# chanchanchan97/ICAFusion

Measured on AMD Instinct MI355X. Metric: RGB/IR image-pairs/sec (two-stream forward + NMS), higher is better.
Workload: dtype bf16

## Files before the change

### icafusion_amd/csrc/api.hip

```cpp
#include "icaf_common.h"
#include <cstring>

namespace icaf {
std::string& last_error() {
    static thread_local std::string e;
    return e;
}
int fail(int code, const char* fmt, ...) {
    char buf[1024];
    va_list ap;
    va_start(ap, fmt);
    vsnprintf(buf, sizeof(buf), fmt, ap);
    va_end(ap);
    last_error() = buf;
    return code;
}
LibOptions g_opt;
}

using namespace icaf;

extern "C" const char* icaf_last_error(void) { return last_error().c_str(); }

extern "C" int icaf_set_option(const char* name, int value) {
    if (!name) return fail(ICAF_ERR_ARG, "icaf_set_option: null name");
    if (!strcmp(name, "detect_elementwise")) g_opt.detect_elementwise = value;
    else if (!strcmp(name, "attn_qsplit")) g_opt.attn_qsplit = value;
    else if (!strcmp(name, "sppf_vpb")) g_opt.sppf_vpb = value;
    else if (!strcmp(name, "letterbox_direct")) g_opt.letterbox_direct = value;
    else if (!strcmp(name, "index64")) g_opt.index64 = value;
    else if (!strcmp(name, "attn_stream")) g_opt.attn_stream = value;
    else if (!strcmp(name, "area_direct")) g_opt.area_direct = value;
    else return fail(ICAF_ERR_ARG, "icaf_set_option: unknown option '%s' (detect_elementwise, attn_qsplit, sppf_vpb, letterbox_direct, index64, attn_stream, area_direct)", name);
    return ICAF_OK;
}
extern "C" int icaf_version(void) { return 100; }

extern "C" int icaf_device_info(int* cu_count, int* lds_bytes, char* arch, int arch_len) {
    int dev = 0;
    ICAF_HIP(hipGetDevice(&dev));
    hipDeviceProp_t prop;
    ICAF_HIP(hipGetDeviceProperties(&prop, dev));
    if (cu_count) *cu_count = prop.multiProcessorCount;
    if (lds_bytes) *lds_bytes = (int)prop.sharedMemPerBlock;
    if (arch && arch_len > 0) {
        strncpy(arch, prop.gcnArchName, arch_len - 1);
        arch[arch_len - 1] = 0;
    }
    return ICAF_OK;
}

extern "C" int icaf_graph_begin(icaf_stream_t s) {
    ICAF_HIP(hipStreamBeginCapture(S(s), hipStreamCaptureModeThreadLocal));
    return ICAF_OK;
}
extern "C" int icaf_graph_end(icaf_stream_t s, void** graph_exec) {
    hipGraph_t graph = nullptr;
    ICAF_HIP(hipStreamEndCapture(S(s), &graph));
    hipGraphExec_t exec = nullptr;
    hipError_t e = hipGraphInstantiate(&exec, graph, nullptr, nullptr, 0);
    hipGraphDestroy(graph);
    if (e != hipSuccess) return fail(ICAF_ERR_HIP, "hipGraphInstantiate -> %s", hipGetErrorString(e));
    *graph_exec = (void*)exec;
    return ICAF_OK;
}
extern "C" int icaf_graph_launch(void* graph_exec, icaf_stream_t s) {
    ICAF_HIP(hipGraphLaunch((hipGraphExec_t)graph_exec, S(s)));
    return ICAF_OK;
}
extern "C" int icaf_graph_destroy(void* graph_exec) {
    if (graph_exec) ICAF_HIP(hipGraphExecDestroy((hipGraphExec_t)graph_exec));
    return ICAF_OK;
}
extern "C" int icaf_event_create(void** ev) {
    hipEvent_t e;
    ICAF_HIP(hipEventCreate(&e));
    *ev = (void*)e;
    return ICAF_OK;
}
extern "C" int icaf_event_record(void* ev, icaf_stream_t s) {
    ICAF_HIP(hipEventRecord((hipEvent_t)ev, S(s)));
    return ICAF_OK;
}
extern "C" int icaf_stream_wait_event(icaf_stream_t s, void* ev) {
    ICAF_HIP(hipStreamWaitEvent(S(s), (hipEvent_t)ev, 0));
    return ICAF_OK;
// ... 15 lines not shown
```

### icafusion_amd/csrc/dmff_wide.hip

```cpp
#include <type_traits>
#include "icaf_common.h"
#include "conv_common.h"

namespace icaf {

struct WideP {
    const void* x;
    const void* att;
    float* part;
    const float* x32;
    float* y32;
    void* qkv;
    void* y;
    const void* wqkv; const float* bqkv;
    const void* wo; const float* bo;
    const void* w1; const float* b1;
    const void* w2; const float* b2;
    const float* ln_a_g[2]; const float* ln_a_b[2];
    const float* ln_m_g; const float* ln_m_b;
    long long wqkv_gs, bqkv_gs, wo_gs, bo_gs, w1_gs, b1_gs, w2_gs, b2_gs, x_gs, y_gs;
    long long rows;
    int C, Kp, Kp4, hid, ldy;
    int qkv_npass;
    float eps_a, eps_m;
    float c_res_a[2], c_acc_a[2], c_res_m[2], c_acc_m[2];
};

constexpr int WROWS = 64;
constexpr int WDEPTH = 4;
template <int NW_, int SL_> struct WG {
    static constexpr int NW = NW_, SL = SL_;
    static constexpr int WT = 64 * NW;
    static constexpr int WPASS = 32 * NW;
    template <int DT> static constexpr int kstep() { return 32 / Elem<DT>::BYTES; }
    template <int DT> static constexpr int ksl() { return kstep<DT>() * SL; }
    template <int DT> static constexpr int nsl2() { return WPASS / ksl<DT>(); }
    static constexpr int TPR = WT / WROWS;
};
using WG8 = WG<8, 4>;
using WG4 = WG<4, 2>;

struct WCursor {
    const u32x4* base;
    int left, seg;
};

template <int WSL, class NEXT>
__device__ __forceinline__ void wfetch(u32x4 (&w)[WSL], WCursor& c, const NEXT& next) {
    if (c.left == 0) return;
#pragma unroll
    for (int k = 0; k < WSL; ++k) w[k] = c.base[k * 64];
    c.base += WSL * 64;
    if (--c.left == 0) { ++c.seg; next(c); }
}

template <int DT, int WSL, class NEXT>
__device__ __forceinline__ void wpass(f32x16 (&acc)[2], const unsigned char* A, int SA, int n, u32x4 (&wq)[WDEPTH][WSL], WCursor& c, const NEXT& next) {
    const int lane = threadIdx.x & 63, l31 = lane & 31, hi = lane >> 5;
    const unsigned char* a0 = A + (size_t)l31 * SA + hi * 16;
    const unsigned char* a1 = a0 + (size_t)32 * SA;
    for (int s = 0; s < n; s += WDEPTH) {
#pragma unroll
        for (int u = 0; u < WDEPTH; ++u) {
#pragma unroll
            for (int k = 0; k < WSL; ++k) {
                const int off = ((s + u) * WSL + k) * 32;
                const u32x4 x0 = *(const u32x4*)(a0 + off);
                const u32x4 x1 = *(const u32x4*)(a1 + off);
                mma_step<DT>(acc[0], wq[u][k], x0);
                mma_step<DT>(acc[1], wq[u][k], x1);
            }
            wfetch<WSL>(wq[u], c, next);
            __builtin_amdgcn_sched_barrier(0);
        }
    }
}

template <int DT, int TPR>
__device__ __forceinline__ void wide_tile_layernorm(unsigned char* tile, int S, int C, const float* __restrict__ gam, const float* __restrict__ bet, float eps) {
    using E = Elem<DT>;
    const int tid = threadIdx.x, row = tid / TPR, part = tid % TPR;
    const int nv = C / E::VEC;
    unsigned char* r = tile + (size_t)row * S;
    float s = 0.0f;
    for (int v = part; v < nv; v += TPR) {
        float t[E::VEC];
        unpack16<DT>(*(const u32x4*)(r + v * 16), t);
#pragma unroll
        for (int j = 0; j < E::VEC; ++j) s += t[j];
    }
    s += __shfl_xor(s, 1); s += __shfl_xor(s, 2);
    if constexpr (TPR == 8) s += __shfl_xor(s, 4);
    const float mean = s / (float)C;
    float q = 0.0f;
    for (int v = part; v < nv; v += TPR) {
        float t[E::VEC];
        unpack16<DT>(*(const u32x4*)(r + v * 16), t);
#pragma unroll
        for (int j = 0; j < E::VEC; ++j) { const float d = t[j] - mean; q += d * d; }
    }
    q += __shfl_xor(q, 1); q += __shfl_xor(q, 2);
    if constexpr (TPR == 8) q += __shfl_xor(q, 4);
    const float rstd = 1.0f / sqrtf(q / (float)C + eps);
    for (int v = part; v < nv; v += TPR) {
        float t[E::VEC], o[E::VEC];
        unpack16<DT>(*(const u32x4*)(r + v * 16), t);
#pragma unroll
        for (int j = 0; j < E::VEC; ++j) o[j] = (t[j] - mean) * rstd * gam[v * E::VEC + j] + bet[v * E::VEC + j];
        *(u32x4*)(r + v * 16) = pack16<DT>(o);
    }
}

__device__ __forceinline__ void wide_place(int bid, int& g, int& idx) { g = (bid & 7) >> 2; idx = (bid >> 3) * 4 + (bid & 3); }
template <int KS> __device__ __forceinline__ void wide_place_ks(int bid, int& g, int& ks, int& idx) {
    const int x = bid & 7, per = 4 / KS;
    g = x >> 2;
    ks = (x & 3) / per;
    idx = (bid >> 3) * per + (x & 3) % per;
}

template <int DT, class G = WG8>
__global__ __launch_bounds__(G::WT) void dmff_wide_ln_qkv_kernel(const WideP p) {
    using E = Elem<DT>;
    using T = typename E::type;
    constexpr int VEC = E::VEC, EB = E::BYTES;
    extern __shared__ __attribute__((aligned(16))) unsigned char smem[];
    const int C = p.C, SA = C * EB + 16;
    unsigned char* tile = smem;
    const int tid = threadIdx.x, lane = tid & 63, l31 = lane & 31, hi = lane >> 5;
    const int wn = __builtin_amdgcn_readfirstlane(tid >> 6);
    const int npass = p.qkv_npass;
    const int ngrp = 3 * (C / G::WPASS) / npass;
    const int ntiles = (int)((p.rows + WROWS - 1) / WROWS);
    int g, idx;
    wide_place(blockIdx.x, g, idx);
    if (idx >= ntiles * ngrp) return;
    const int tile_i = idx / ngrp, grp = idx - tile_i * ngrp;
    const long long r0 = (long long)tile_i * WROWS;
    const int ks_row = p.Kp / G::template kstep<DT>(), nsl = C / G::template ksl<DT>();

    const u32x4* wf = (const u32x4*)((const T*)p.wqkv + g * p.wqkv_gs) + lane;
    auto next = [&](WCursor& c) {
        if (c.seg >= npass) { c.left = 0; return; }
        c.base = wf + (long long)((grp * npass + c.seg) * G::NW + wn) * ks_row * 64;
        c.left = nsl;
    };
    WCursor cur; cur.seg = 0; next(cur);
    u32x4 wq[WDEPTH][G::SL];
#pragma unroll
    for (int u = 0; u < WDEPTH; ++u) wfetch<G::SL>(wq[u], cur, next);

    {
        const T* xg = (const T*)p.x + g * p.x_gs;
        const int nv = C / VEC;
        for (int i = tid; i < WROWS * nv; i += G::WT) {
            const int row = i / nv, v = i - row * nv;
            long long r = r0 + row;
            r = r < p.rows ? r : p.rows - 1;
            *(u32x4*)(tile + (size_t)row * SA + v * 16) = *(const u32x4*)(xg + r * C + v * VEC);
        }
    }
    lds_barrier();
    wide_tile_layernorm<DT, G::TPR>(tile, SA, C, p.ln_a_g[g], p.ln_a_b[g], p.eps_a);
    lds_barrier();

    const float* bias = p.bqkv + g * p.bqkv_gs;
    const int nout = 3 * C;
    T* out = (T*)p.qkv + (long long)g * p.rows * nout;
    for (int j = 0; j < npass; ++j) {
        f32x16 acc[2];
#pragma unroll
        for (int t = 0; t < 2; ++t)
#pragma unroll
            for (int r = 0; r < 16; ++r) acc[t][r] = 0.0f;
        wpass<DT, G::SL>(acc, tile, SA, nsl, wq, cur, next);
        const int nb = (grp * npass + j) * G::WPASS + wn * 32;
#pragma unroll
        for (int t = 0; t < 2; ++t) {
            const long long row = r0 + t * 32 + l31;
            if (row < p.rows) {
#pragma unroll
                for (int q = 0; q < 4; ++q) {
                    const int n = nb + 8 * q + 4 * hi;
                    const f32x4 b = *(const f32x4*)(bias + n);
                    *(typename Quad<DT>::type*)(out + row * nout + n) =
                        pack4<DT>(acc[t][4 * q] + b[0], acc[t][4 * q + 1] + b[1], acc[t][4 * q + 2] + b[2], acc[t][4 * q + 3] + b[3]);
                }
            }
        }
    }
}

template <int DT, int NPW, int KS = 1, class G = WG8, bool R32 = false>
__global__ __launch_bounds__(G::WT) void dmff_wide_proj_mlp_kernel(const WideP p) {
    using E = Elem<DT>;
    using T = typename E::type;
    constexpr int VEC = E::VEC, EB = E::BYTES;
    extern __shared__ __attribute__((aligned(16))) unsigned char smem[];
    const int C = p.C, SA = C * EB + 16;
    constexpr int WPASS = G::WPASS, WT = G::WT, NSL2 = G::template nsl2<DT>(), KST = G::template kstep<DT>();
    constexpr int SH = WPASS * EB + 16;
    unsigned char* T0 = smem;
    unsigned char* Hb = T0 + (size_t)WROWS * SA;
    float* red = (float*)(Hb + (size_t)WROWS * SH);
    float* b1s = red + G::NW * 64;

    const int tid = threadIdx.x, lane = tid & 63, l31 = lane & 31, hi = lane >> 5;
    const int wn = __builtin_amdgcn_readfirstlane(tid >> 6);
    const int ntiles = (int)((p.rows + WROWS - 1) / WROWS);
    int g, tile_i, ksl = 0;
    if constexpr (KS == 1) wide_place(blockIdx.x, g, tile_i);
    else wide_place_ks<KS>(blockIdx.x, g, ksl, tile_i);
    if (tile_i >= ntiles) return;
    const long long r0 = (long long)tile_i * WROWS;
    const int ks_row = p.Kp / KST, ks_row4 = p.Kp4 / KST, nsl = C / G::template ksl<DT>(), nchunk = p.hid / WPASS / KS, chunk0 = ksl * nchunk;

    const u32x4* wof = (const u32x4*)((const T*)p.wo + g * p.wo_gs) + lane;
    const u32x4* w1f = (const u32x4*)((const T*)p.w1 + g * p.w1_gs) + lane;
    const u32x4* w2f = (const u32x4*)((const T*)p.w2 + g * p.w2_gs) + lane;
    auto next = [&](WCursor& c) {
        const int s = c.seg;
        if (s < NPW) { c.base = wof + (long long)(s * G::NW + wn) * ks_row * 64; c.left = nsl; return; }
        const int m = s - NPW, chunk = m / (1 + NPW), r = m - chunk * (1 + NPW);
        if (chunk >= nchunk) { c.left = 0; return; }
        if (r == 0) { c.base = w1f + (long long)((chunk0 + chunk) * G::NW + wn) * ks_row * 64; c.left = nsl; }
        else { c.base = w2f + ((long long)((r - 1) * G::NW + wn) * ks_row4 + (chunk0 + chunk) * (WPASS / KST)) * 64; c.left = NSL2; }
    };
    WCursor cur; cur.seg = 0; next(cur);
    u32x4 wq[WDEPTH][G::SL];
#pragma unroll
    for (int u = 0; u < WDEPTH; ++u) wfetch<G::SL>(wq[u], cur, next);

    {
        const T* att = (const T*)p.att + (long long)g * p.rows * C;
        const int nv = C / VEC;
        for (int i = tid; i < WROWS * nv; i += WT) {
            const int row = i / nv, v = i - row * nv;
            long long r = r0 + row;
            r = r < p.rows ? r : p.rows - 1;
            *(u32x4*)(T0 + (size_t)row * SA + v * 16) = *(const u32x4*)(att + r * C + v * VEC);
        }
        const float* b1 = p.b1 + g * p.b1_gs;
        for (int i = tid; i < p.hid / KS; i += WT) b1s[i] = b1[chunk0 * WPASS + i];
    }
    lds_barrier();

    bool rok[2];
    const T* xres[2];
    T* yrow[2];
    const float* x32row[2];
    float* y32row[2];
#pragma unroll
    for (int t = 0; t < 2; ++t) {
        const long long row = r0 + t * 32 + l31;
        rok[t] = row < p.rows;
        const long long grow = rok[t] ? row : p.rows - 1;
        xres[t] = (const T*)p.x + g * p.x_gs + grow * C;
        yrow[t] = (T*)p.y + g * p.y_gs + grow * p.ldy;
        x32row[t] = (R32 && p.x32) ? p.x32 + ((long long)g * p.rows + grow) * C : nullptr;
        y32row[t] = R32 ? p.y32 + ((long long)g * p.rows + grow) * C : nullptr;
    }
    using XQ = typename std::conditional<R32, f32x4, typename Quad<DT>::type>::type;
    auto xq_pack = [](float a, float b, float c, float d) -> XQ {
        if constexpr (R32) return f32x4{a, b, c, d};
        else return pack4<DT>(a, b, c, d);
    };
    auto xq_unpack = [](const XQ& q, float* f) {
        if constexpr (R32) { f[0] = q[0]; f[1] = q[1]; f[2] = q[2]; f[3] = q[3]; }
        else unpack4<DT>(q, f);
    };

    constexpr bool PARK = NPW >= 2 || KS > 1;
    XQ xatt[NPW][2][4];
    {
        const float* bias = p.bo + g * p.bo_gs;
        const float ca = p.c_acc_a[g], cr = p.c_res_a[g];
#pragma unroll
        for (int i = 0; i < NPW; ++i) {
            f32x16 acc[2];
#pragma unroll
            for (int t = 0; t < 2; ++t)
#pragma unroll
                for (int r = 0; r < 16; ++r) acc[t][r] = 0.0f;
            wpass<DT, G::SL>(acc, T0, SA, nsl, wq, cur, next);
#pragma unroll
            for (int t = 0; t < 2; ++t)
#pragma unroll
                for (int q = 0; q < 4; ++q) {
                    const int n = i * WPASS + wn * 32 + 8 * q + 4 * hi;
                    const f32x4 bv = *(const f32x4*)(bias + n);
                    float rv[4], v[4];
                    if (R32 && x32row[t]) { const f32x4 r4 = *(const f32x4*)(x32row[t] + n); rv[0] = r4[0]; rv[1] = r4[1]; rv[2] = r4[2]; rv[3] = r4[3]; }
                    else unpack4<DT>(*(const typename Quad<DT>::type*)(xres[t] + n), rv);
#pragma unroll
                    for (int j = 0; j < 4; ++j) v[j] = __builtin_fmaf(cr, rv[j], (acc[t][4 * q + j] + bv[j]) * ca);
                    xatt[i][t][q] = xq_pack(v[0], v[1], v[2], v[3]);
                }
        }
    }
    {
        float mean[2], rstd[2];
        float sum[2] = {0.0f, 0.0f};
#pragma unroll
        for (int i = 0; i < NPW; ++i)
#pragma unroll
            for (int t = 0; t < 2; ++t)
#pragma unroll
                for (int q = 0; q < 4; ++q) {
                    float v[4];
                    xq_unpack(xatt[i][t][q], v);
                    sum[t] += (v[0] + v[1]) + (v[2] + v[3]);
                }
#pragma unroll
        for (int t = 0; t < 2; ++t) {
            sum[t] += __shfl_xor(sum[t], 32);
            if (hi == 0) red[wn * 64 + t * 32 + l31] = sum[t];
        }
        lds_barrier();
#pragma unroll
        for (int t = 0; t < 2; ++t) {
            float s = 0.0f;
#pragma unroll
            for (int w = 0; w < G::NW; ++w) s += red[w * 64 + t * 32 + l31];
            mean[t] = s / (float)C;
        }
        lds_barrier();
        float sq[2] = {0.0f, 0.0f};
#pragma unroll
        for (int i = 0; i < NPW; ++i)
#pragma unroll
            for (int t = 0; t < 2; ++t)
#pragma unroll
                for (int q = 0; q < 4; ++q) {
                    float v[4];
                    xq_unpack(xatt[i][t][q], v);
#pragma unroll
                    for (int j = 0; j < 4; ++j) { const float d = v[j] - mean[t]; sq[t] += d * d; }
                }
#pragma unroll
        for (int t = 0; t < 2; ++t) {
            sq[t] += __shfl_xor(sq[t], 32);
            if (hi == 0) red[wn * 64 + t * 32 + l31] = sq[t];
        }
        lds_barrier();
#pragma unroll
        for (int t = 0; t < 2; ++t) {
            float s = 0.0f;
#pragma unroll
            for (int w = 0; w < G::NW; ++w) s += red[w * 64 + t * 32 + l31];
            rstd[t] = 1.0f / sqrtf(s / (float)C + p.eps_m);
        }
#pragma unroll
        for (int i = 0; i < NPW; ++i)
#pragma unroll
            for (int q = 0; q < 4; ++q) {
                const int n = i * WPASS + wn * 32 + 8 * q + 4 * hi;
                const f32x4 gv = *(const f32x4*)(p.ln_m_g + n), bv = *(const f32x4*)(p.ln_m_b + n);
#pragma unroll
                for (int t = 0; t < 2; ++t) {
                    float v[4], o[4];
                    xq_unpack(xatt[i][t][q], v);
#pragma unroll
                    for (int j = 0; j < 4; ++j) o[j] = (v[j] - mean[t]) * rstd[t] * gv[j] + bv[j];
                    *(typename Quad<DT>::type*)(T0 + (size_t)(t * 32 + l31) * SA + n * EB) = pack4<DT>(o[0], o[1], o[2], o[3]);
                    if constexpr (PARK) {
                        if (rok[t] && ksl == 0) {
                            if constexpr (R32) *(f32x4*)(y32row[t] + n) = xatt[i][t][q];
                            else *(typename Quad<DT>::type*)(yrow[t] + n) = xatt[i][t][q];
                        }
                    }
                }
            }
        lds_barrier();
    }
    f32x16 acc2[NPW][2];
#pragma unroll
    for (int i = 0; i < NPW; ++i)
#pragma unroll
        for (int t = 0; t < 2; ++t)
#pragma unroll
            for (int r = 0; r < 16; ++r) acc2[i][t][r] = 0.0f;
    for (int chunk = 0; chunk < nchunk; ++chunk) {
        f32x16 acc[2];
#pragma unroll
        for (int t = 0; t < 2; ++t)
#pragma unroll
            for (int r = 0; r < 16; ++r) acc[t][r] = 0.0f;
        wpass<DT, G::SL>(acc, T0, SA, nsl, wq, cur, next);
        lds_barrier();
#pragma unroll
        for (int t = 0; t < 2; ++t)
#pragma unroll
            for (int q = 0; q < 4; ++q) {
                const int nl = wn * 32 + 8 * q + 4 * hi;
                const f32x4 bv = *(const f32x4*)(b1s + chunk * WPASS + nl);
                *(typename Quad<DT>::type*)(Hb + (size_t)(t * 32 + l31) * SH + nl * EB) =
                    pack4<DT>(apply_act<ICAF_ACT_GELU, DT>(acc[t][4 * q] + bv[0]), apply_act<ICAF_ACT_GELU, DT>(acc[t][4 * q + 1] + bv[1]),
                              apply_act<ICAF_ACT_GELU, DT>(acc[t][4 * q + 2] + bv[2]), apply_act<ICAF_ACT_GELU, DT>(acc[t][4 * q + 3] + bv[3]));
            }
        lds_barrier();
#pragma unroll
        for (int i = 0; i < NPW; ++i) wpass<DT, G::SL>(acc2[i], Hb, SH, NSL2, wq, cur, next);
    }
    if constexpr (KS > 1) {
        float* part = p.part + ((long long)(ksl * 2 + g) * p.rows) * C;
#pragma unroll
        for (int i = 0; i < NPW; ++i)
#pragma unroll
            for (int q = 0; q < 4; ++q) {
                const int n = i * WPASS + wn * 32 + 8 * q + 4 * hi;
#pragma unroll
                for (int t = 0; t < 2; ++t)
                    if (rok[t])
                        *(f32x4*)(part + (r0 + t * 32 + l31) * C + n) = f32x4{acc2[i][t][4 * q], acc2[i][t][4 * q + 1], acc2[i][t][4 * q + 2], acc2[i][t][4 * q + 3]};
            }
    } else {
        const float* b2 = p.b2 + g * p.b2_gs;
        const float ca = p.c_acc_m[g], cr = p.c_res_m[g];
#pragma unroll
        for (int i = 0; i < NPW; ++i)
#pragma unroll
            for (int q = 0; q < 4; ++q) {
                const int n = i * WPASS + wn * 32 + 8 * q + 4 * hi;
                const f32x4 bv = *(const f32x4*)(b2 + n);
#pragma unroll
                for (int t = 0; t < 2; ++t) {
                    float rv[4], v[4];
                    if constexpr (PARK && R32) { const f32x4 r4 = *(const f32x4*)(y32row[t] + n); rv[0] = r4[0]; rv[1] = r4[1]; rv[2] = r4[2]; rv[3] = r4[3]; }
                    else if constexpr (PARK) unpack4<DT>(*(const typename Quad<DT>::type*)(yrow[t] + n), rv);
                    else xq_unpack(xatt[i][t][q], rv);
#pragma unroll
                    for (int j = 0; j < 4; ++j) v[j] = __builtin_fmaf(cr, rv[j], (acc2[i][t][4 * q + j] + bv[j]) * ca);
                    if (rok[t]) {
                        *(typename Quad<DT>::type*)(yrow[t] + n) = pack4<DT>(v[0], v[1], v[2], v[3]);
                        if constexpr (R32) *(f32x4*)(y32row[t] + n) = f32x4{v[0], v[1], v[2], v[3]};
                    }
                }
            }
    }
}

template <int DT, int KS, bool R32 = false>
__global__ __launch_bounds__(256) void dmff_wide_reduce_kernel(const WideP p) {
    using T = typename Elem<DT>::type;
    const int C = p.C, nq = C >> 2;
    const long long total = 2 * p.rows * nq;
    for (long long idx = (long long)blockIdx.x * 256 + threadIdx.x; idx < total; idx += (long long)gridDim.x * 256) {
        const int qn = (int)(idx % nq);
        const long long gr = idx / nq;
        const int g = (int)(gr / p.rows);
        const long long row = gr - (long long)g * p.rows;
        const int n = qn * 4;
        f32x4 sum = *(const f32x4*)(p.part + ((long long)g * p.rows + row) * C + n);
#pragma unroll
        for (int k = 1; k < KS; ++k) {
            const f32x4 v = *(const f32x4*)(p.part + ((long long)(k * 2 + g) * p.rows + row) * C + n);
            sum[0] += v[0]; sum[1] += v[1]; sum[2] += v[2]; sum[3] += v[3];
        }
        const f32x4 bv = *(const f32x4*)(p.b2 + g * p.b2_gs + n);
        T* y = (T*)p.y + g * p.y_gs + row * p.ldy + n;
        float* y32 = R32 ? p.y32 + ((long long)g * p.rows + row) * C + n : nullptr;
        float rv[4], v[4];
        if constexpr (R32) { const f32x4 r4 = *(const f32x4*)y32; rv[0] = r4[0]; rv[1] = r4[1]; rv[2] = r4[2]; rv[3] = r4[3]; }
        else unpack4<DT>(*(const typename Quad<DT>::type*)y, rv);
        const float ca = p.c_acc_m[g], cr = p.c_res_m[g];
#pragma unroll
        for (int j = 0; j < 4; ++j) v[j] = __builtin_fmaf(cr, rv[j], (sum[j] + bv[j]) * ca);
        *(typename Quad<DT>::type*)y = pack4<DT>(v[0], v[1], v[2], v[3]);
        if constexpr (R32) *(f32x4*)y32 = f32x4{v[0], v[1], v[2], v[3]};
    }
}

static int wide_fill(const icaf_dmff_args* a, WideP& p, const char* who) {
    if (!a || !a->x) return fail(ICAF_ERR_ARG, "%s: null pointer", who);
    if (a->dtype != ICAF_BF16 && a->dtype != ICAF_F16 && !(a->dtype == ICAF_F32 && a->C == 128))
        return fail(ICAF_ERR_UNSUPPORTED, "%s: 16-bit types (fp32: the C = 128 parity build only; dtype %d, C = %d)", who, a->dtype, a->C);
    if (a->B < 1 || a->N < 1) return fail(ICAF_ERR_ARG, "%s: bad B/N", who);
    if (a->C != 128 && a->C != 256 && a->C != 512) return fail(ICAF_ERR_UNSUPPORTED, "%s: C=%d (built for 128 [four wavefronts, 128-channel passes] and 256 / 512 [eight, 256-channel passes])", who, a->C);
    if (a->Kp < a->C || a->Kp % (a->dtype == ICAF_F32 ? 32 : 64)) return fail(ICAF_ERR_ARG, "%s: Kp=%d", who, a->Kp);
    p.x = a->x; p.qkv = a->qkv; p.y = a->y; p.att = nullptr; p.part = nullptr;
    p.x32 = a->x32; p.y32 = a->y32;
    if (a->x32 && !a->y32) return fail(ICAF_ERR_ARG, "%s: x32 without y32 (the fp32 residual stream is read AND written by every iteration but the first)", who);
    if (a->y32 && a->dtype == ICAF_F32) return fail(ICAF_ERR_ARG, "%s: the fp32 residual stream belongs to the 16-bit builds", who);
    if ((a->x32 && ((uintptr_t)a->x32 & 15)) || (a->y32 && ((uintptr_t)a->y32 & 15))) return fail(ICAF_ERR_ARG, "%s: x32 / y32 must be 16-byte aligned", who);
    p.wqkv = a->wqkv; p.bqkv = a->bqkv; p.wo = a->wo; p.bo = a->bo; p.w1 = a->w1; p.b1 = a->b1; p.w2 = a->w2; p.b2 = a->b2;
    p.ln_a_g[0] = a->ln_attn_gamma[0]; p.ln_a_g[1] = a->ln_attn_gamma[1]; p.ln_a_b[0] = a->ln_attn_beta[0]; p.ln_a_b[1] = a->ln_attn_beta[1];
    p.ln_m_g = a->ln_mlp_gamma; p.ln_m_b = a->ln_mlp_beta;
    p.wqkv_gs = a->wqkv_gs; p.bqkv_gs = a->bqkv_gs; p.wo_gs = a->wo_gs; p.bo_gs = a->bo_gs; p.w1_gs = a->w1_gs; p.b1_gs = a->b1_gs;
    p.w2_gs = a->w2_gs; p.b2_gs = a->b2_gs; p.x_gs = a->x_gs; p.y_gs = a->y_gs;
    p.rows = (long long)a->B * a->N; p.C = a->C; p.Kp = a->Kp; p.Kp4 = a->Kp4; p.hid = a->hidden; p.ldy = a->ldy;
    p.qkv_npass = a->reserved == 1 ? 1 : 3;
    p.eps_a = a->eps_attn; p.eps_m = a->eps_mlp;
    for (int g = 0; g < 2; ++g) {
        p.c_res_a[g] = a->coef_res_attn[g]; p.c_acc_a[g] = a->coef_acc_attn[g];
        p.c_res_m[g] = a->coef_res_mlp[g]; p.c_acc_m[g] = a->coef_acc_mlp[g];
    }
    return ICAF_OK;
}

template <int DT, class G>
static int launch_wide_ln_qkv(const WideP& p, hipStream_t s) {
    const size_t lds = (size_t)WROWS * (p.C * Elem<DT>::BYTES + 16);
    ICAF_LDS_OPTIN((dmff_wide_ln_qkv_kernel<DT, G>), lds);
    const long long work = ((p.rows + WROWS - 1) / WROWS) * (3 * (p.C / G::WPASS) / p.qkv_npass);
    hipLaunchKernelGGL((dmff_wide_ln_qkv_kernel<DT, G>), dim3((unsigned)(8 * ((work + 3) / 4))), dim3(G::WT), lds, s, p);
    ICAF_LAUNCH_CHECK();
    return ICAF_OK;
}

template <class G>
static size_t wide_proj_mlp_lds(int C, int hid, int eb = 2) {
    return (size_t)WROWS * (C * eb + 16) + (size_t)WROWS * (G::WPASS * eb + 16) + G::NW * 64 * sizeof(float) + (size_t)hid * sizeof(float);
}

template <int DT, int NPW, class G, bool R32 = false>
static int launch_wide_proj_mlp(const WideP& p, hipStream_t s) {
    const size_t lds = wide_proj_mlp_lds<G>(p.C, p.hid, Elem<DT>::BYTES);
    ICAF_LDS_OPTIN((dmff_wide_proj_mlp_kernel<DT, NPW, 1, G, R32>), lds);
    const long long ntiles = (p.rows + WROWS - 1) / WROWS;
    hipLaunchKernelGGL((dmff_wide_proj_mlp_kernel<DT, NPW, 1, G, R32>), dim3((unsigned)(8 * ((ntiles + 3) / 4))), dim3(G::WT), lds, s, p);
    ICAF_LAUNCH_CHECK();
    return ICAF_OK;
}

template <int DT, int NPW, int KS, bool R32 = false>
static int launch_wide_proj_mlp_split(const WideP& p, hipStream_t s) {
    const size_t lds = wide_proj_mlp_lds<WG8>(p.C, p.hid / KS);
    ICAF_LDS_OPTIN((dmff_wide_proj_mlp_kernel<DT, NPW, KS, WG8, R32>), lds);
    const long long ntiles = (p.rows + WROWS - 1) / WROWS, per = 4 / KS;
    hipLaunchKernelGGL((dmff_wide_proj_mlp_kernel<DT, NPW, KS, WG8, R32>), dim3((unsigned)(8 * ((ntiles + per - 1) / per))), dim3(WG8::WT), lds, s, p);
    ICAF_LAUNCH_CHECK();
    return ICAF_OK;
}

template <int DT>
static int dispatch_wide_split(const WideP& p, int ksplit, hipStream_t s) {
    if (p.y32) {
        if (ksplit != 2) return fail(ICAF_ERR_UNSUPPORTED, "icaf_dmff_wide_proj_mlp_split: the fp32 residual stream is built for ksplit = 2");
        return p.C == 256 ? launch_wide_proj_mlp_split<DT, 1, 2, true>(p, s) : launch_wide_proj_mlp_split<DT, 2, 2, true>(p, s);
    }
    if (p.C == 256) return ksplit == 2 ? launch_wide_proj_mlp_split<DT, 1, 2>(p, s) : launch_wide_proj_mlp_split<DT, 1, 4>(p, s);
    return ksplit == 2 ? launch_wide_proj_mlp_split<DT, 2, 2>(p, s) : launch_wide_proj_mlp_split<DT, 2, 4>(p, s);
}

template <int DT>
static int dispatch_wide_ln_qkv(const WideP& p, hipStream_t s) {
    return p.C == 128 ? launch_wide_ln_qkv<DT, WG4>(p, s) : launch_wide_ln_qkv<DT, WG8>(p, s);
}

template <int DT>
static int dispatch_wide_proj_mlp(const WideP& p, hipStream_t s) {
    if (p.y32) {
        if (p.C == 128) return launch_wide_proj_mlp<DT, 1, WG4, true>(p, s);
        if (p.C == 256) return launch_wide_proj_mlp<DT, 1, WG8, true>(p, s);
        return fail(ICAF_ERR_UNSUPPORTED, "icaf_dmff_wide_proj_mlp: the fp32 residual stream at C = 512 is built for the hidden split (ksplit = 2) only");
    }
    if (p.C == 128) return launch_wide_proj_mlp<DT, 1, WG4>(p, s);
    return p.C == 256 ? launch_wide_proj_mlp<DT, 1, WG8>(p, s) : launch_wide_proj_mlp<DT, 2, WG8>(p, s);
}

template <int DT>
static int launch_wide_reduce(const WideP& p, int ksplit, hipStream_t s) {
    const long long items = 2 * p.rows * (p.C / 4);
    long long blocks = (items + 255) / 256;
    if (blocks > 4096) blocks = 4096;
    if (p.y32) {
        if (ksplit != 2) return fail(ICAF_ERR_UNSUPPORTED, "icaf_dmff_wide_reduce: the fp32 residual stream is built for ksplit = 2");
        hipLaunchKernelGGL((dmff_wide_reduce_kernel<DT, 2, true>), dim3((unsigned)blocks), dim3(256), 0, s, p);
    } else if (ksplit == 2) hipLaunchKernelGGL((dmff_wide_reduce_kernel<DT, 2>), dim3((unsigned)blocks), dim3(256), 0, s, p);
    else hipLaunchKernelGGL((dmff_wide_reduce_kernel<DT, 4>), dim3((unsigned)blocks), dim3(256), 0, s, p);
    ICAF_LAUNCH_CHECK();
    return ICAF_OK;
}

}

using namespace icaf;

extern "C" int icaf_dmff_wide_ln_qkv(const icaf_dmff_args* a, icaf_stream_t s) {
    WideP p{};
    int st = wide_fill(a, p, "icaf_dmff_wide_ln_qkv");
    if (st) return st;
    if (!a->qkv || !a->wqkv || !a->bqkv || !a->ln_attn_gamma[0] || !a->ln_attn_gamma[1] || !a->ln_attn_beta[0] || !a->ln_attn_beta[1])
// ... 44 lines not shown
```

### icafusion_amd/csrc/icaf_common.h

```cpp
#pragma once
#include <hip/hip_runtime.h>
#include <stdint.h>
#include <string>
#include <cstdio>
#include <cstdarg>
#include <atomic>
#include "../../include/icaf.h"

namespace icaf {

std::string& last_error();
int fail(int code, const char* fmt, ...);
struct LibOptions { int detect_elementwise = 0, attn_qsplit = 0, sppf_vpb = 0, letterbox_direct = 0, index64 = 0, attn_stream = 0, area_direct = 0; };
extern LibOptions g_opt;

#define ICAF_HIP(expr)                                                                        \
    do {                                                                                      \
        hipError_t _e = (expr);                                                               \
        if (_e != hipSuccess)                                                                 \
            return icaf::fail(ICAF_ERR_HIP, "%s -> %s (%s:%d)", #expr, hipGetErrorString(_e), \
                              __FILE__, __LINE__);                                            \
    } while (0)

#define ICAF_LAUNCH_CHECK() ICAF_HIP(hipGetLastError())

using u32x4 = __attribute__((ext_vector_type(4))) unsigned int;
using u32x2 = __attribute__((ext_vector_type(2))) unsigned int;
using f32x4 = __attribute__((ext_vector_type(4))) float;
using f32x16 = __attribute__((ext_vector_type(16))) float;
using bf16x8 = __attribute__((ext_vector_type(8))) __bf16;
using f16x8 = __attribute__((ext_vector_type(8))) _Float16;

__device__ __forceinline__ float bf16_to_f32(unsigned short h) { return __uint_as_float(((unsigned int)h) << 16); }
__device__ __forceinline__ unsigned short f32_to_bf16(float f) {
    return __builtin_bit_cast(unsigned short, (__bf16)f);
}
__device__ __forceinline__ unsigned int pack2_bf16(float lo, float hi) {
    using bf16x2 = __attribute__((ext_vector_type(2))) __bf16;
    bf16x2 v = {(__bf16)lo, (__bf16)hi};
    return __builtin_bit_cast(unsigned int, v);
}
__device__ __forceinline__ unsigned int pack2_f16(float lo, float hi) {
    using f16x2 = __attribute__((ext_vector_type(2))) _Float16;
    f16x2 v = {(_Float16)lo, (_Float16)hi};
    return __builtin_bit_cast(unsigned int, v);
}
__device__ __forceinline__ float f16_to_f32(unsigned short h) {
    _Float16 v = __builtin_bit_cast(_Float16, h);
    return (float)v;
}
__device__ __forceinline__ unsigned short f32_to_f16(float f) {
    _Float16 v = (_Float16)f;
    return __builtin_bit_cast(unsigned short, v);
}

template <int DT> struct Elem;
template <> struct Elem<ICAF_F32> {
    using type = float;
    static constexpr int VEC = 4;
    static constexpr int BYTES = 4;
    static __device__ __forceinline__ float ld(const float* p) { return *p; }
    static __device__ __forceinline__ void st(float* p, float v) { *p = v; }
};
template <> struct Elem<ICAF_BF16> {
    using type = unsigned short;
    static constexpr int VEC = 8;
// ... 139 lines not shown
```

### icafusion_amd/ops.py

```python
import collections
import contextlib
import ctypes as C
import weakref

import numpy as np
import torch

from . import _lib
from .options import OPT
from ._lib import BneckArgs, ConvArgs, DmffArgs, FrameGeom, Stem2Args, check, lib, F32, BF16, F16, ACT_NONE, ACT_SILU, ACT_GELU, ACT_RELU

_DT = {torch.float32: F32, torch.bfloat16: BF16, torch.float16: F16}
VEC = {torch.float32: 4, torch.bfloat16: 8, torch.float16: 8}
N_ALIGN = 128
K_ALIGN_BYTES = 128


def dtype_code(dt):
    try:
        return _DT[dt]
    except KeyError:
        raise _lib.IcafError(f"unsupported dtype {dt}; supported: float32, bfloat16, float16") from None


# ... 623 lines not shown
    a.coef_res_mlp[0], a.coef_res_mlp[1] = co[4], co[6]
    a.coef_acc_mlp[0], a.coef_acc_mlp[1] = co[5], co[7]
    return a


def dmff_ln_qkv(x, qkv, packs, ln, coef, eps, B, N, heads, name="dmff_ln_qkv"):
    a = _dmff_args(x, qkv, None, packs, ln, coef, eps, B, N, heads)
    rows, Cc = x.shape[1], x.shape[2]
    es = x.element_size()
    return Launch(lib().icaf_dmff_ln_qkv, (C.byref(a),), keep=(a, x, qkv, packs, ln), name=name, flops=2.0 * 2 * rows * Cc * 3 * Cc,
                  nbytes=2 * (rows * Cc * es + 3 * Cc * Cc * es + rows * 3 * Cc * es))


def dmff_attn_mlp(x, qkv, y, packs, ln, coef, eps, B, N, heads, name="dmff_attn_mlp"):
    a = _dmff_args(x, qkv, y, packs, ln, coef, eps, B, N, heads)
    rows, Cc = x.shape[1], x.shape[2]
    es, hid = x.element_size(), coef["hidden"]
    flops = 2.0 * (B * heads * 4.0 * N * N * (Cc // heads)) + 2.0 * 2 * rows * (Cc * Cc + 2 * Cc * hid)
    nbytes = 2 * (rows * 3 * Cc * es + 2 * rows * Cc * es + (Cc * Cc + 2 * Cc * hid) * es)
    return Launch(lib().icaf_dmff_attn_mlp, (C.byref(a),), keep=(a, x, qkv, y, packs, ln), name=name, flops=flops, nbytes=nbytes)


def dmff_wide_ok(C_, hidden, dt):
    wpass = 128 if C_ == 128 else 256
    es = 4 if dt == torch.float32 else 2
    lds = 64 * (C_ * es + 16) + 64 * (wpass * es + 16) + 8 * 64 * 4 + hidden * 4
    if dt == torch.float32:
        return C_ == 128 and hidden % wpass == 0 and lds <= 160 * 1024
    return dt in (torch.bfloat16, torch.float16) and C_ in (128, 256, 512) and hidden % wpass == 0 and lds <= 160 * 1024


def _wide_packs(packs):
    return {k: ((frag_weights(v[0]), v[1], v[2]) if k in ("qkv", "out", "fc1", "fc2") else v) for k, v in packs.items()}


def dmff_wide_ln_qkv(x, qkv, packs, ln, coef, eps, B, N, heads, name="dmff_ln_qkv"):
    wp = _wide_packs(packs)
    a = _dmff_args(x, qkv, None, wp, ln, coef, eps, B, N, heads)
    a.reserved = OPT.dmff_qkv_npass
    rows, Cc = x.shape[1], x.shape[2]
    es = x.element_size()
    return Launch(lib().icaf_dmff_wide_ln_qkv, (C.byref(a),), keep=(a, x, qkv, wp, packs, ln), name=name, flops=2.0 * 2 * rows * Cc * 3 * Cc,
                  nbytes=2 * (rows * Cc * es + 3 * Cc * Cc * es + rows * 3 * Cc * es))


def dmff_wide_ksplit(N, C_, hidden):
    if C_ < 256:
        return 1
    if OPT.dmff_ksplit:
        return OPT.dmff_ksplit if hidden % (256 * OPT.dmff_ksplit) == 0 else 1
    return 2 if (9 * C_ * C_ * 2 > 3 * 2 ** 20 and N <= 128 and hidden % 512 == 0) else 1


def dmff_wide_proj_mlp(x, att, y, packs, ln, coef, eps, B, N, heads, name="dmff_proj_mlp", partial=None, ksplit=1, x32=None, y32=None):
    rows, Cc = x.shape[1], x.shape[2]
    assert att.shape == (2, rows, Cc) and att.is_contiguous() and att.dtype == x.dtype
    wp = _wide_packs(packs)
    a = _dmff_args(x, None, y, wp, ln, coef, eps, B, N, heads)
    es, hid = x.element_size(), coef["hidden"]
    flops = 2.0 * 2 * rows * (Cc * Cc + 2 * Cc * hid)
    nbytes = 2 * (3 * rows * Cc * es + (Cc * Cc + 2 * Cc * hid) * es)
    if y32 is not None:
        for t in (x32, y32):
            assert t is None or (t.dtype == torch.float32 and t.shape == (2, rows, Cc) and t.is_contiguous())
        a.y32 = y32.data_ptr()
        a.x32 = x32.data_ptr() if x32 is not None else None
        nbytes += (2 if x32 is not None else 1) * 2 * rows * Cc * 4
    else:
        assert x32 is None
    if ksplit > 1:
        assert partial is not None and partial.dtype == torch.float32 and partial.is_contiguous() and partial.shape == (ksplit, 2, rows, Cc)
        flops += 2.0 * 2 * rows * Cc * Cc * (ksplit - 1)
        nbytes += partial.numel() * 4
        main = Launch(lib().icaf_dmff_wide_proj_mlp_split, (C.byref(a), att.data_ptr(), partial.data_ptr(), int(ksplit)),
                      keep=(a, x, att, y, wp, packs, ln, partial, x32, y32), name=name, flops=flops, nbytes=nbytes)
        red = Launch(lib().icaf_dmff_wide_reduce, (C.byref(a), partial.data_ptr(), int(ksplit)), keep=(a, y, partial, wp, packs, y32),
                     name=name + "_reduce", nbytes=partial.numel() * 4 + 2 * 2 * rows * Cc * es)
        return [main, red]
    return Launch(lib().icaf_dmff_wide_proj_mlp, (C.byref(a), att.data_ptr()), keep=(a, x, att, y, wp, packs, ln, x32, y32), name=name, flops=flops, nbytes=nbytes)


def dmff_upsample_merge(tokens, fea_rgb, fea_ir, out, th, tw, name="dmff_upsample_merge"):
    B, H, W, Cc, ld0 = _act_geom(fea_rgb)
    ld1 = _act_geom(fea_ir)[4]
    Bo, Ho, Wo, Co, ldo = _act_geom(out)
    assert (Bo, Ho, Wo, Co) == (B, H, W, 2 * Cc) and tokens.shape == (2, B * th * tw, Cc)
    nb = (2 * fea_rgb.numel() + out.numel()) * out.element_size()
    return Launch(lib().icaf_dmff_upsample_merge,
                  (tokens.data_ptr(), fea_rgb.data_ptr(), ld0, fea_ir.data_ptr(), ld1, out.data_ptr(), ldo,
                   dtype_code(out.dtype), B, H, W, Cc, th, tw), keep=(tokens, fea_rgb, fea_ir, out), name=name,
                  nbytes=nb)


def detect_decode(p, z, logits, raw, na, no, row_offset, stride, anchors_px, name="detect_decode"):
    B, ny, nx, cp, ldp = _act_geom(p)
    assert p.dtype == torch.float32 and z.dtype == torch.float32 and z.is_contiguous()
    arr = (C.c_float * (2 * na))(*[float(v) for v in anchors_px])
    nb = p.numel() * 4 + 3 * B * na * ny * nx * no * 4
    return Launch(lib().icaf_detect_decode,
                  (p.data_ptr(), ldp, z.data_ptr(), logits.data_ptr() if logits is not None else None,
                   raw.data_ptr() if raw is not None else None, B, ny, nx, na, no, z.shape[1], row_offset,
                   float(stride), arr), keep=(p, z, logits, raw, arr), name=name, nbytes=nb)


def detect_decode_kernel(p, z, raw, na, no):
    B, ny, nx, cp, ldp = _act_geom(p)
# ... 500 lines not shown
```

Measured before the change: 16900.

## Pipeline DMFF MLP fc1 with GELU epilogue and prefetch LDS A-fragments ahead

Software-pipelines the fused proj+MLP kernel so the next chunk's fc1 MFMA pass runs interleaved with the GELU epilogue of the previous chunk, using sched_group_barrier to mix MFMA and VALU work. The weight cursor is reordered to fetch fc1 weights one chunk ahead. wpass also gains a register ring that prefetches A fragments from LDS a few steps ahead. Launch bounds now declare occupancy hints (4 and 2). The price is extra register pressure from double accumulators, with a possible spill or occupancy loss; a serial fallback option is kept.

Result: no change. 16900 (median of 2 runs) (-0.0%).

```diff
diff --git a/icafusion_amd/csrc/api.hip b/icafusion_amd/csrc/api.hip
--- a/icafusion_amd/csrc/api.hip
+++ b/icafusion_amd/csrc/api.hip
@@ -31,7 +31,8 @@
     else if (!strcmp(name, "index64")) g_opt.index64 = value;
     else if (!strcmp(name, "attn_stream")) g_opt.attn_stream = value;
     else if (!strcmp(name, "area_direct")) g_opt.area_direct = value;
-    else return fail(ICAF_ERR_ARG, "icaf_set_option: unknown option '%s' (detect_elementwise, attn_qsplit, sppf_vpb, letterbox_direct, index64, attn_stream, area_direct)", name);
+    else if (!strcmp(name, "dmff_mlp_serial")) g_opt.dmff_mlp_serial = value;
+    else return fail(ICAF_ERR_ARG, "icaf_set_option: unknown option '%s' (detect_elementwise, attn_qsplit, sppf_vpb, letterbox_direct, index64, attn_stream, area_direct, dmff_mlp_serial)", name);
     return ICAF_OK;
 }
 extern "C" int icaf_version(void) { return 100; }
diff --git a/icafusion_amd/csrc/dmff_wide.hip b/icafusion_amd/csrc/dmff_wide.hip
--- a/icafusion_amd/csrc/dmff_wide.hip
+++ b/icafusion_amd/csrc/dmff_wide.hip
@@ -1,6 +1,10 @@
 #include <type_traits>
 #include "icaf_common.h"
 #include "conv_common.h"
+
+#ifndef ICAF_DMFF_AHEAD
+#define ICAF_DMFF_AHEAD 1
+#endif
 
 namespace icaf {
 
@@ -54,25 +58,77 @@
     if (--c.left == 0) { ++c.seg; next(c); }
 }
 
-template <int DT, int WSL, class NEXT>
+__device__ __forceinline__ void wfrag(u32x4 (&x)[2], const unsigned char* a0, const unsigned char* a1, int step) {
+    x[0] = *(const u32x4*)(a0 + step * 32);
+    x[1] = *(const u32x4*)(a1 + step * 32);
+}
+
+template <int DT, int WSL, int AH, class NEXT>
 __device__ __forceinline__ void wpass(f32x16 (&acc)[2], const unsigned char* A, int SA, int n, u32x4 (&wq)[WDEPTH][WSL], WCursor& c, const NEXT& next) {
+    static_assert(AH == 0 || WSL % AH == 0, "the ring index of a step must be a compile-time constant");
     const int lane = threadIdx.x & 63, l31 = lane & 31, hi = lane >> 5;
     const unsigned char* a0 = A + (size_t)l31 * SA + hi * 16;
     const unsigned char* a1 = a0 + (size_t)32 * SA;
+    constexpr int R = AH ? AH : 1;
+    u32x4 xf[R][2];
+#pragma unroll
+    for (int j = 0; j < AH; ++j) wfrag(xf[j], a0, a1, j);
     for (int s = 0; s < n; s += WDEPTH) {
 #pragma unroll
         for (int u = 0; u < WDEPTH; ++u) {
 #pragma unroll
             for (int k = 0; k < WSL; ++k) {
-                const int off = ((s + u) * WSL + k) * 32;
-                const u32x4 x0 = *(const u32x4*)(a0 + off);
-                const u32x4 x1 = *(const u32x4*)(a1 + off);
-                mma_step<DT>(acc[0], wq[u][k], x0);
-                mma_step<DT>(acc[1], wq[u][k], x1);
+                const int j = (s + u) * WSL + k;
+                if constexpr (AH == 0) wfrag(xf[0], a0, a1, j);
+                mma_step<DT>(acc[0], wq[u][k], xf[k % R][0]);
+                mma_step<DT>(acc[1], wq[u][k], xf[k % R][1]);
+                if constexpr (AH != 0) {
+                    if (k + AH < WSL || u + 1 < WDEPTH || s + WDEPTH < n) wfrag(xf[k % R], a0, a1, j + AH);
+                }
             }
             wfetch<WSL>(wq[u], c, next);
             __builtin_amdgcn_sched_barrier(0);
         }
+    }
+}
+
+template <int DT>
+__device__ __forceinline__ void gelu_quad(const f32x16 (&acc)[2], int i, const float* b1c, unsigned char* hrow, int SH) {
+    const int t = i >> 2, q = i & 3;
+    const f32x4 bv = *(const f32x4*)(b1c + 8 * q);
+    *(typename Quad<DT>::type*)(hrow + (size_t)(t * 32) * SH + 8 * q * Elem<DT>::BYTES) =
+        pack4<DT>(apply_act<ICAF_ACT_GELU, DT>(acc[t][4 * q] + bv[0]), apply_act<ICAF_ACT_GELU, DT>(acc[t][4 * q + 1] + bv[1]),
+                  apply_act<ICAF_ACT_GELU, DT>(acc[t][4 * q + 2] + bv[2]), apply_act<ICAF_ACT_GELU, DT>(acc[t][4 * q + 3] + bv[3]));
+}
+
+template <int DT, int WSL, int NS, class NEXT>
+__device__ __forceinline__ void wpass_gelu(f32x16 (&acc)[2], const unsigned char* A, int SA, u32x4 (&wq)[WDEPTH][WSL], WCursor& c, const NEXT& next,
+                                           const f32x16 (&gacc)[2], const float* b1c, unsigned char* hrow, int SH) {
+    static_assert(NS % WDEPTH == 0 && 8 % NS == 0, "slices of an fc1 pass");
+    constexpr int QPS = 8 / NS;
+    constexpr int NM = 2 * WSL * (DT == ICAF_F32 ? 4 : 1);
+    constexpr int VPM = (QPS * (DT == ICAF_F32 ? 400 : 48) + NM - 1) / NM;
+    const int lane = threadIdx.x & 63, l31 = lane & 31, hi = lane >> 5;
+    const unsigned char* a0 = A + (size_t)l31 * SA + hi * 16;
+    const unsigned char* a1 = a0 + (size_t)32 * SA;
+#pragma unroll
+    for (int s = 0; s < NS; ++s) {
+#pragma unroll
+        for (int k = 0; k < WSL; ++k) {
+            u32x4 xf[2];
+            wfrag(xf, a0, a1, s * WSL + k);
+            mma_step<DT>(acc[0], wq[s % WDEPTH][k], xf[0]);
+            mma_step<DT>(acc[1], wq[s % WDEPTH][k], xf[1]);
+        }
+#pragma unroll
+        for (int j = 0; j < QPS; ++j) gelu_quad<DT>(gacc, s * QPS + j, b1c, hrow, SH);
+#pragma unroll
+        for (int m = 0; m < NM; ++m) {
+            __builtin_amdgcn_sched_group_barrier(0x008, 1, 0);
+            __builtin_amdgcn_sched_group_barrier(0x002, VPM, 0);
+        }
+        wfetch<WSL>(wq[s % WDEPTH], c, next);
+        __builtin_amdgcn_sched_barrier(0);
     }
 }
 
@@ -120,12 +176,13 @@
 }
 
 template <int DT, class G = WG8>
-__global__ __launch_bounds__(G::WT) void dmff_wide_ln_qkv_kernel(const WideP p) {
+__global__ __launch_bounds__(G::WT, 4) void dmff_wide_ln_qkv_kernel(const WideP p) {
     using E = Elem<DT>;
     using T = typename E::type;
     constexpr int VEC = E::VEC, EB = E::BYTES;
     extern __shared__ __attribute__((aligned(16))) unsigned char smem[];
     const int C = p.C, SA = C * EB + 16;
+    constexpr int AHQ = !ICAF_DMFF_AHEAD ? 0 : G::NW == 8 ? 2 : G::SL;
     unsigned char* tile = smem;
     const int tid = threadIdx.x, lane = tid & 63, l31 = lane & 31, hi = lane >> 5;
     const int wn = __builtin_amdgcn_readfirstlane(tid >> 6);
@@ -173,7 +230,7 @@
         for (int t = 0; t < 2; ++t)
 #pragma unroll
             for (int r = 0; r < 16; ++r) acc[t][r] = 0.0f;
-        wpass<DT, G::SL>(acc, tile, SA, nsl, wq, cur, next);
+        wpass<DT, G::SL, AHQ>(acc, tile, SA, nsl, wq, cur, next);
         const int nb = (grp * npass + j) * G::WPASS + wn * 32;
 #pragma unroll
         for (int t = 0; t < 2; ++t) {
@@ -191,8 +248,8 @@
     }
 }
 
-template <int DT, int NPW, int KS = 1, class G = WG8, bool R32 = false>
-__global__ __launch_bounds__(G::WT) void dmff_wide_proj_mlp_kernel(const WideP p) {
+template <int DT, int NPW, int KS = 1, class G = WG8, bool R32 = false, bool SERIAL = false>
+__global__ __launch_bounds__(G::WT, 2) void dmff_wide_proj_mlp_kernel(const WideP p) {
     using E = Elem<DT>;
     using T = typename E::type;
     constexpr int VEC = E::VEC, EB = E::BYTES;
@@ -200,6 +257,8 @@
     const int C = p.C, SA = C * EB + 16;
     constexpr int WPASS = G::WPASS, WT = G::WT, NSL2 = G::template nsl2<DT>(), KST = G::template kstep<DT>();
     constexpr int SH = WPASS * EB + 16;
+    constexpr int AH = ICAF_DMFF_AHEAD ? G::SL : 0;
+    constexpr bool PIPE = !SERIAL && NPW == 1;
     unsigned char* T0 = smem;
     unsigned char* Hb = T0 + (size_t)WROWS * SA;
     float* red = (float*)(Hb + (size_t)WROWS * SH);
@@ -219,12 +278,22 @@
     const u32x4* w1f = (const u32x4*)((const T*)p.w1 + g * p.w1_gs) + lane;
     const u32x4* w2f = (const u32x4*)((const T*)p.w2 + g * p.w2_gs) + lane;
     auto next = [&](WCursor& c) {
-        const int s = c.seg;
+        int s = c.seg;
         if (s < NPW) { c.base = wof + (long long)(s * G::NW + wn) * ks_row * 64; c.left = nsl; return; }
-        const int m = s - NPW, chunk = m / (1 + NPW), r = m - chunk * (1 + NPW);
+        auto fc1 = [&](int chunk) { c.base = w1f + (long long)((chunk0 + chunk) * G::NW + wn) * ks_row * 64; c.left = nsl; };
+        if constexpr (PIPE) {
+            if (s == NPW) { fc1(0); return; }
+            s -= 1;
+        }
+        int m = s - NPW, chunk = m / (1 + NPW), r = m - chunk * (1 + NPW);
         if (chunk >= nchunk) { c.left = 0; return; }
-        if (r == 0) { c.base = w1f + (long long)((chunk0 + chunk) * G::NW + wn) * ks_row * 64; c.left = nsl; }
-        else { c.base = w2f + ((long long)((r - 1) * G::NW + wn) * ks_row4 + (chunk0 + chunk) * (WPASS / KST)) * 64; c.left = NSL2; }
+        if constexpr (PIPE) {
+            if (r == 0) {
+                if (chunk + 1 < nchunk) { fc1(chunk + 1); return; }
+                ++c.seg; r = 1;
+            }
+        } else if (r == 0) { fc1(chunk); return; }
+        c.base = w2f + ((long long)((r - 1) * G::NW + wn) * ks_row4 + (chunk0 + chunk) * (WPASS / KST)) * 64; c.left = NSL2;
     };
     WCursor cur; cur.seg = 0; next(cur);
     u32x4 wq[WDEPTH][G::SL];
@@ -247,19 +316,16 @@
 
     bool rok[2];
     const T* xres[2];
-    T* yrow[2];
     const float* x32row[2];
-    float* y32row[2];
+    auto grow = [&](int t) { const long long row = r0 + t * 32 + l31; return row < p.rows ? row : p.rows - 1; };
 #pragma unroll
     for (int t = 0; t < 2; ++t) {
-        const long long row = r0 + t * 32 + l31;
-        rok[t] = row < p.rows;
-        const long long grow = rok[t] ? row : p.rows - 1;
-        xres[t] = (const T*)p.x + g * p.x_gs + grow * C;
-        yrow[t] = (T*)p.y + g * p.y_gs + grow * p.ldy;
-        x32row[t] = (R32 && p.x32) ? p.x32 + ((long long)g * p.rows + grow) * C : nullptr;
-        y32row[t] = R32 ? p.y32 + ((long long)g * p.rows + grow) * C : nullptr;
-    }
+        rok[t] = r0 + t * 32 + l31 < p.rows;
+        xres[t] = (const T*)p.x + g * p.x_gs + grow(t) * C;
+        x32row[t] = (R32 && p.x32) ? p.x32 + ((long long)g * p.rows + grow(t)) * C : nullptr;
+    }
+    auto yrow = [&](int t) { return (T*)p.y + g * p.y_gs + grow(t) * p.ldy; };
+    auto y32row = [&](int t) { return p.y32 + ((long long)g * p.rows + grow(t)) * C; };
     using XQ = typename std::conditional<R32, f32x4, typename Quad<DT>::type>::type;
     auto xq_pack = [](float a, float b, float c, float d) -> XQ {
         if constexpr (R32) return f32x4{a, b, c, d};
@@ -282,7 +348,7 @@
             for (int t = 0; t < 2; ++t)
 #pragma unroll
                 for (int r = 0; r < 16; ++r) acc[t][r] = 0.0f;
-            wpass<DT, G::SL>(acc, T0, SA, nsl, wq, cur, next);
+            wpass<DT, G::SL, AH>(acc, T0, SA, nsl, wq, cur, next);
 #pragma unroll
             for (int t = 0; t < 2; ++t)
 #pragma unroll
@@ -365,8 +431,8 @@
                     *(typename Quad<DT>::type*)(T0 + (size_t)(t * 32 + l31) * SA + n * EB) = pack4<DT>(o[0], o[1], o[2], o[3]);
                     if constexpr (PARK) {
                         if (rok[t] && ksl == 0) {
-                            if constexpr (R32) *(f32x4*)(y32row[t] + n) = xatt[i][t][q];
-                            else *(typename Quad<DT>::type*)(yrow[t] + n) = xatt[i][t][q];
+                            if constexpr (R32) *(f32x4*)(y32row(t) + n) = xatt[i][t][q];
+                            else *(typename Quad<DT>::type*)(yrow(t) + n) = xatt[i][t][q];
                         }
                     }
                 }
@@ -380,27 +446,48 @@
         for (int t = 0; t < 2; ++t)
 #pragma unroll
             for (int r = 0; r < 16; ++r) acc2[i][t][r] = 0.0f;
-    for (int chunk = 0; chunk < nchunk; ++chunk) {
-        f32x16 acc[2];
+    const float* b1c = b1s + wn * 32 + 4 * hi;
+    unsigned char* hrow = Hb + (size_t)l31 * SH + (wn * 32 + 4 * hi) * EB;
+    auto zero = [](f32x16 (&a)[2]) {
 #pragma unroll
         for (int t = 0; t < 2; ++t)
 #pragma unroll
-            for (int r = 0; r < 16; ++r) acc[t][r] = 0.0f;
-        wpass<DT, G::SL>(acc, T0, SA, nsl, wq, cur, next);
-        lds_barrier();
-#pragma unroll
-        for (int t = 0; t < 2; ++t)
-#pragma unroll
-            for (int q = 0; q < 4; ++q) {
-                const int nl = wn * 32 + 8 * q + 4 * hi;
-                const f32x4 bv = *(const f32x4*)(b1s + chunk * WPASS + nl);
-                *(typename Quad<DT>::type*)(Hb + (size_t)(t * 32 + l31) * SH + nl * EB) =
-                    pack4<DT>(apply_act<ICAF_ACT_GELU, DT>(acc[t][4 * q] + bv[0]), apply_act<ICAF_ACT_GELU, DT>(acc[t][4 * q + 1] + bv[1]),
-                              apply_act<ICAF_ACT_GELU, DT>(acc[t][4 * q + 2] + bv[2]), apply_act<ICAF_ACT_GELU, DT>(acc[t][4 * q + 3] + bv[3]));
+            for (int r = 0; r < 16; ++r) a[t][r] = 0.0f;
+    };
+    if constexpr (!PIPE) {
+        for (int chunk = 0; chunk < nchunk; ++chunk) {
+            f32x16 acc[2];
+            zero(acc);
+            wpass<DT, G::SL, AH>(acc, T0, SA, nsl, wq, cur, next);
+            lds_barrier();
+#pragma unroll
+            for (int i = 0; i < 8; ++i) gelu_quad<DT>(acc, i, b1c + chunk * WPASS, hrow, SH);
+            lds_barrier();
+#pragma unroll
+            for (int i = 0; i < NPW; ++i) wpass<DT, G::SL, AH>(acc2[i], Hb, SH, NSL2, wq, cur, next);
+        }
+    } else {
+        constexpr int NS1 = NPW * NSL2;
+        f32x16 acc1[2][2];
+        auto step = [&](f32x16 (&ga)[2], f32x16 (&na)[2], int chunk) {
+            lds_barrier();
+            if (chunk + 1 < nchunk) {
+                zero(na);
+                wpass_gelu<DT, G::SL, NS1>(na, T0, SA, wq, cur, next, ga, b1c + chunk * WPASS, hrow, SH);
+            } else {
+#pragma unroll
+                for (int i = 0; i < 8; ++i) gelu_quad<DT>(ga, i, b1c + chunk * WPASS, hrow, SH);
             }
-        lds_barrier();
-#pragma unroll
-        for (int i = 0; i < NPW; ++i) wpass<DT, G::SL>(acc2[i], Hb, SH, NSL2, wq, cur, next);
+            lds_barrier();
+#pragma unroll
+            for (int i = 0; i < NPW; ++i) wpass<DT, G::SL, AH>(acc2[i], Hb, SH, NSL2, wq, cur, next);
+        };
+        zero(acc1[0]);
+        wpass<DT, G::SL, AH>(acc1[0], T0, SA, nsl, wq, cur, next);
+        for (int chunk = 0; chunk < nchunk; chunk += 2) {
+            step(acc1[0], acc1[1], chunk);
+            if (chunk + 1 < nchunk) step(acc1[1], acc1[0], chunk + 1);
+        }
     }
     if constexpr (KS > 1) {
         float* part = p.part + ((long long)(ksl * 2 + g) * p.rows) * C;
@@ -426,14 +513,14 @@
 #pragma unroll
                 for (int t = 0; t < 2; ++t) {
                     float rv[4], v[4];
-                    if constexpr (PARK && R32) { const f32x4 r4 = *(const f32x4*)(y32row[t] + n); rv[0] = r4[0]; rv[1] = r4[1]; rv[2] = r4[2]; rv[3] = r4[3]; }
-                    else if constexpr (PARK) unpack4<DT>(*(const typename Quad<DT>::type*)(yrow[t] + n), rv);
+                    if constexpr (PARK && R32) { const f32x4 r4 = *(const f32x4*)(y32row(t) + n); rv[0] = r4[0]; rv[1] = r4[1]; rv[2] = r4[2]; rv[3] = r4[3]; }
+                    else if constexpr (PARK) unpack4<DT>(*(const typename Quad<DT>::type*)(yrow(t) + n), rv);
                     else xq_unpack(xatt[i][t][q], rv);
 #pragma unroll
                     for (int j = 0; j < 4; ++j) v[j] = __builtin_fmaf(cr, rv[j], (acc2[i][t][4 * q + j] + bv[j]) * ca);
                     if (rok[t]) {
-                        *(typename Quad<DT>::type*)(yrow[t] + n) = pack4<DT>(v[0], v[1], v[2], v[3]);
-                        if constexpr (R32) *(f32x4*)(y32row[t] + n) = f32x4{v[0], v[1], v[2], v[3]};
+                        *(typename Quad<DT>::type*)(yrow(t) + n) = pack4<DT>(v[0], v[1], v[2], v[3]);
+                        if constexpr (R32) *(f32x4*)(y32row(t) + n) = f32x4{v[0], v[1], v[2], v[3]};
                     }
                 }
             }
@@ -513,22 +600,28 @@
     return (size_t)WROWS * (C * eb + 16) + (size_t)WROWS * (G::WPASS * eb + 16) + G::NW * 64 * sizeof(float) + (size_t)hid * sizeof(float);
 }
 
-template <int DT, int NPW, class G, bool R32 = false>
+template <int DT, int NPW, class G, bool R32 = false, bool SERIAL = false>
 static int launch_wide_proj_mlp(const WideP& p, hipStream_t s) {
+    if constexpr (!SERIAL && NPW == 1) {
+        if (g_opt.dmff_mlp_serial) return launch_wide_proj_mlp<DT, NPW, G, R32, true>(p, s);
+    }
     const size_t lds = wide_proj_mlp_lds<G>(p.C, p.hid, Elem<DT>::BYTES);
-    ICAF_LDS_OPTIN((dmff_wide_proj_mlp_kernel<DT, NPW, 1, G, R32>), lds);
+    ICAF_LDS_OPTIN((dmff_wide_proj_mlp_kernel<DT, NPW, 1, G, R32, SERIAL>), lds);
     const long long ntiles = (p.rows + WROWS - 1) / WROWS;
-    hipLaunchKernelGGL((dmff_wide_proj_mlp_kernel<DT, NPW, 1, G, R32>), dim3((unsigned)(8 * ((ntiles + 3) / 4))), dim3(G::WT), lds, s, p);
+    hipLaunchKernelGGL((dmff_wide_proj_mlp_kernel<DT, NPW, 1, G, R32, SERIAL>), dim3((unsigned)(8 * ((ntiles + 3) / 4))), dim3(G::WT), lds, s, p);
     ICAF_LAUNCH_CHECK();
     return ICAF_OK;
 }
 
-template <int DT, int NPW, int KS, bool R32 = false>
+template <int DT, int NPW, int KS, bool R32 = false, bool SERIAL = false>
 static int launch_wide_proj_mlp_split(const WideP& p, hipStream_t s) {
+    if constexpr (!SERIAL && NPW == 1) {
+        if (g_opt.dmff_mlp_serial) return launch_wide_proj_mlp_split<DT, NPW, KS, R32, true>(p, s);
+    }
     const size_t lds = wide_proj_mlp_lds<WG8>(p.C, p.hid / KS);
-    ICAF_LDS_OPTIN((dmff_wide_proj_mlp_kernel<DT, NPW, KS, WG8, R32>), lds);
+    ICAF_LDS_OPTIN((dmff_wide_proj_mlp_kernel<DT, NPW, KS, WG8, R32, SERIAL>), lds);
     const long long ntiles = (p.rows + WROWS - 1) / WROWS, per = 4 / KS;
-    hipLaunchKernelGGL((dmff_wide_proj_mlp_kernel<DT, NPW, KS, WG8, R32>), dim3((unsigned)(8 * ((ntiles + per - 1) / per))), dim3(WG8::WT), lds, s, p);
+    hipLaunchKernelGGL((dmff_wide_proj_mlp_kernel<DT, NPW, KS, WG8, R32, SERIAL>), dim3((unsigned)(8 * ((ntiles + per - 1) / per))), dim3(WG8::WT), lds, s, p);
     ICAF_LAUNCH_CHECK();
     return ICAF_OK;
 }
diff --git a/icafusion_amd/csrc/icaf_common.h b/icafusion_amd/csrc/icaf_common.h
--- a/icafusion_amd/csrc/icaf_common.h
+++ b/icafusion_amd/csrc/icaf_common.h
@@ -11,7 +11,11 @@
 
 std::string& last_error();
 int fail(int code, const char* fmt, ...);
-struct LibOptions { int detect_elementwise = 0, attn_qsplit = 0, sppf_vpb = 0, letterbox_direct = 0, index64 = 0, attn_stream = 0, area_direct = 0; };
+#ifndef ICAF_DMFF_MLP_SERIAL
+#define ICAF_DMFF_MLP_SERIAL 0
+#endif
+struct LibOptions { int detect_elementwise = 0, attn_qsplit = 0, sppf_vpb = 0, letterbox_direct = 0, index64 = 0, attn_stream = 0, area_direct = 0,
+                        dmff_mlp_serial = ICAF_DMFF_MLP_SERIAL; };
 extern LibOptions g_opt;
 
 #define ICAF_HIP(expr)                                                                        \
diff --git a/icafusion_amd/ops.py b/icafusion_amd/ops.py
--- a/icafusion_amd/ops.py
+++ b/icafusion_amd/ops.py
@@ -699,6 +699,15 @@
     return 2 if (9 * C_ * C_ * 2 > 3 * 2 ** 20 and N <= 128 and hidden % 512 == 0) else 1
 
 
+@contextlib.contextmanager
+def dmff_mlp_serial(on=True):
+    check(lib().icaf_set_option(b"dmff_mlp_serial", int(bool(on))), "icaf_set_option(dmff_mlp_serial)")
+    try:
+        yield
+    finally:
+        check(lib().icaf_set_option(b"dmff_mlp_serial", 0), "icaf_set_option(dmff_mlp_serial)")
+
+
 def dmff_wide_proj_mlp(x, att, y, packs, ln, coef, eps, B, N, heads, name="dmff_proj_mlp", partial=None, ksplit=1, x32=None, y32=None):
     rows, Cc = x.shape[1], x.shape[2]
     assert att.shape == (2, rows, Cc) and att.is_contiguous() and att.dtype == x.dtype
```
